# CliMA/ClimaOcean.jl

Measured on AMD Instinct MI355X. Metric: flux-kernel surface cells/s (update_state!: JRA55 interp + similarity-theory fluxes + net fluxes), higher is better.
Workload: dtype f64

## Files before the change

### climaocean.jl_amd/coflux/abi.py

```python
import ctypes as C
import os

import numpy as np

ABI_VERSION = 5
COMM_ID_BYTES = 128
PEER_HANDLE_BYTES = 64
HALO_NONE, HALO_RCCL, HALO_PEER = 0, 1, 2
FOLD_CENTER, FOLD_X_FACE, FOLD_Y_FACE = 0, 1, 2
SKIN_EXPLICIT, SKIN_SEMI_IMPLICIT, SKIN_LINEARISED = 0, 1, 2

SIMILARITY_LOGARITHMIC, SIMILARITY_COARE_LOGARITHMIC = 0, 1
STABILITY_EDSON2013, STABILITY_SHEBA, STABILITY_LARGE_YEAGER = 0, 1, 2
ROUGHNESS_CONSTANT, ROUGHNESS_CHARNOCK, ROUGHNESS_WIND_CHARNOCK = 0, 1, 2
SCALAR_ROUGHNESS_CONSTANT, SCALAR_ROUGHNESS_REYNOLDS = 0, 1
VISCOSITY_CONSTANT, VISCOSITY_TEMPERATURE_DEPENDENT = 0, 1
STOP_CONVERGENCE, STOP_FIXED = 0, 1
FORMULATION_SIMILARITY, FORMULATION_LARGE_YEAGER = 0, 1
VELOCITY_RELATIVE, VELOCITY_WIND = 0, 1
MASK_NONE, MASK_U8, MASK_BOTTOM_HEIGHT = 0, 1, 2
ALBEDO_CONSTANT, ALBEDO_LATITUDE_DEPENDENT = 0, 1
OPT_SOLVER, OPT_TRIP_HINTS, OPT_FUSED_NET, OPT_ICE_ORBIT_SHORTCUT, OPT_MERGED_PREFETCH = 0, 3, 6, 7, 9
OPT_INTERP_TILE_CAP, OPT_AO_CHUNK = 1, 4
OPT_INTERP_TILE_ROWS = 15
# ... 285 lines not shown
    "cf_device_alloc", "cf_device_free", "cf_h2d", "cf_d2h",
    "cf_interpolate_atmosphere_state", "cf_compute_atmosphere_ocean_fluxes",
    "cf_compute_net_ocean_fluxes", "cf_update_state", "cf_normalize_salinity_flux",
    "cf_default_sea_ice_params", "cf_set_sea_ice_formulation", "cf_compute_atmosphere_sea_ice_fluxes",
    "cf_compute_net_sea_ice_fluxes", "cf_update_state_sea_ice",
    "cf_time_stage", "cf_time_copy", "cf_profile_enable", "cf_profile_read",
    "cf_comm_unique_id", "cf_comm_init", "cf_comm_destroy", "cf_halo_exchange_rows",
    "cf_peer_halo_export", "cf_peer_halo_connect", "cf_halo_exchange_rows_peer", "cf_peer_halo_stats", "cf_fold_north_halo",
    "cf_time_steps", "cf_prefetch_atmosphere_state",
    "cf_default_sea_ice_albedo_params", "cf_set_sea_ice_albedo", "cf_compute_sea_ice_albedo",
    "cf_default_ice_ocean_params", "cf_compute_sea_ice_ocean_fluxes",
    "cf_interpolate_land_freshwater", "cf_set_land_freshwater", "cf_materialize_salinity_restoring",
    "cf_window_create", "cf_window_destroy", "cf_window_host_buffer", "cf_window_wait_slot", "cf_window_commit",
    "cf_window_upload", "cf_window_find", "cf_window_source",
    "cf_ensure_chunk_table", "cf_debug_chunk_table", "cf_debug_interp_grid", "cf_debug_land_zero_launches", "cf_solver_path", "cf_solver_iteration_path", "cf_solver_latency_layout", "cf_comm_count", "cf_build_stamp", "cf_discard_prefetched_atmosphere_state",
    "cf_debug_prefetch_stats",
    "cf_average_create", "cf_average_destroy", "cf_average_reset", "cf_average_collect", "cf_average_weight", "cf_attach_average",
    "cf_average_create_derived", "cf_average_create_budget", "cf_attach_average_slot",
    "cf_integrals_create", "cf_integrals_destroy", "cf_integrals_collect", "cf_integrals_count", "cf_integrals_read",
    "cf_integrals_reset", "cf_attach_integrals",
    "cf_monitor_create", "cf_monitor_destroy", "cf_monitor_collect", "cf_monitor_count", "cf_monitor_read", "cf_monitor_status",
    "cf_monitor_reset", "cf_attach_monitor",
    "cf_climatology_create", "cf_climatology_destroy", "cf_climatology_reset", "cf_climatology_collect", "cf_climatology_weights",
    "cf_climatology_extremes", "cf_calendar_bin", "cf_attach_climatology",
    "cf_regrid_create", "cf_regrid_destroy", "cf_regrid_apply",
    "cf_prepare_coupled_step", "cf_time_steps_coupled",
    "cf_checkpoint_create", "cf_checkpoint_destroy", "cf_checkpoint_add_array", "cf_checkpoint_add_average", "cf_checkpoint_add_climatology",
    "cf_checkpoint_add_integrals", "cf_checkpoint_add_monitor", "cf_checkpoint_set_host_blob", "cf_checkpoint_capture", "cf_checkpoint_wait",
    "cf_checkpoint_restore", "cf_checkpoint_verify", "cf_checkpoint_hash", "cf_checkpoint_host_blob",
)

# ... 101 lines not shown
    lib.cf_peer_halo_connect.argtypes = [vp, vp, vp, C.c_int, C.c_int]
    lib.cf_halo_exchange_rows_peer.argtypes = [vp, C.POINTER(vp), C.c_int, C.c_int]
    lib.cf_fold_north_halo.argtypes = [vp, C.POINTER(vp), C.POINTER(C.c_int), C.POINTER(C.c_double), C.c_int, C.c_int]
    lib.cf_time_steps.argtypes = [
        vp, C.c_int64, C.c_int, C.POINTER(RunSchedule), C.POINTER(AtmosSource), C.POINTER(InterpWeights),
        C.POINTER(InterfaceFluxes), C.POINTER(SeaIceFields), C.POINTER(NetOceanFluxes)]
    lib.cf_prepare_coupled_step.argtypes = [vp, C.POINTER(CoupledPrepare)]
    lib.cf_time_steps_coupled.argtypes = [
        vp, C.c_int64, C.c_int, C.POINTER(RunSchedule), C.POINTER(AtmosSource), C.POINTER(InterpWeights),
        C.POINTER(InterfaceFluxes), C.POINTER(SeaIceFields), C.POINTER(NetOceanFluxes), C.POINTER(CoupledStep)]
    lib.cf_prefetch_atmosphere_state.argtypes = [vp, C.POINTER(AtmosSource), C.POINTER(InterpWeights), C.POINTER(ExchangeFields)]
    lib.cf_ensure_chunk_table.argtypes = [vp, vp]
    lib.cf_debug_chunk_table.argtypes = [vp, C.POINTER(C.c_int), C.POINTER(C.c_int), C.c_int, C.POINTER(C.c_int), C.POINTER(C.c_int)]
    lib.cf_debug_interp_grid.argtypes = [vp, C.POINTER(C.c_int), C.POINTER(C.c_int)]
    lib.cf_debug_land_zero_launches.argtypes = [vp, C.POINTER(C.c_int)]
    lib.cf_solver_path.argtypes = [vp, C.POINTER(C.c_int), C.POINTER(C.c_int)]
    lib.cf_default_sea_ice_albedo_params.argtypes = [C.POINTER(SeaIceAlbedoParams)]
    lib.cf_set_sea_ice_albedo.argtypes = [vp, C.POINTER(SeaIceAlbedoParams)]
    lib.cf_compute_sea_ice_albedo.argtypes = [vp, C.POINTER(SeaIceAlbedoParams), vp, vp, vp, vp]
    lib.cf_default_ice_ocean_params.argtypes = [C.POINTER(IceOceanParams)]
    lib.cf_compute_sea_ice_ocean_fluxes.argtypes = [vp, C.POINTER(IceOceanParams), C.POINTER(OceanSurface), vp, vp, vp,
                                                    C.POINTER(IceOceanFluxes)]
    lib.cf_interpolate_land_freshwater.argtypes = [vp, C.POINTER(LandSource), C.POINTER(InterpWeights), vp]
    lib.cf_set_land_freshwater.argtypes = [vp, vp]
    lib.cf_materialize_salinity_restoring.argtypes = [vp, C.c_double, vp, C.POINTER(OceanSurface), vp]
    lib.cf_window_create.argtypes = [vp, C.c_int32, C.c_int32, C.c_int32, C.POINTER(vp)]
    lib.cf_window_destroy.argtypes = [vp]
    lib.cf_window_host_buffer.argtypes = [vp, C.c_int32, C.c_int32]
    lib.cf_window_host_buffer.restype = C.POINTER(C.c_float)
    lib.cf_window_wait_slot.argtypes = [vp, C.c_int32]
# ... 34 lines not shown
        getattr(lib, "cf_checkpoint_add_" + kind).argtypes = [vp, C.c_char_p, vp]
    lib.cf_checkpoint_set_host_blob.argtypes = [vp, vp, C.c_size_t]
    lib.cf_checkpoint_capture.argtypes = [vp]
    lib.cf_checkpoint_wait.argtypes = [vp, C.POINTER(vp), C.POINTER(C.c_size_t)]
    lib.cf_checkpoint_restore.argtypes = [vp, vp, C.c_size_t]
    lib.cf_checkpoint_verify.argtypes = [vp, C.c_size_t]
    lib.cf_checkpoint_hash.argtypes = [vp, C.c_size_t, C.POINTER(C.c_uint64)]
    lib.cf_checkpoint_host_blob.argtypes = [vp, C.c_size_t, C.POINTER(vp), C.POINTER(C.c_size_t)]
    for name in EXPORTED_SYMBOLS:
        fn = getattr(lib, name)
        if name not in ("cf_last_error", "cf_device_alloc", "cf_window_host_buffer", "cf_build_stamp"):
            fn.restype = C.c_int
    if path is None:
        _lib = lib
    return lib
```

### climaocean.jl_amd/coflux/runtime.py

```python
import ctypes as C

import numpy as np
import torch

from . import abi

EXCHANGE_NAMES = ("u", "v", "T", "p", "q", "Qs", "Ql", "Mp")
FLUX_NAMES = ("sensible_heat", "latent_heat", "water_vapor", "x_momentum", "y_momentum", "temperature")
FLUX_OPTIONAL = ("friction_velocity", "temperature_scale", "humidity_scale")
NET_NAMES = ("u", "v", "T", "S", "shortwave_surface_flux", "upwelling_longwave",
             "downwelling_longwave", "downwelling_shortwave")
ICE_NAMES = ("concentration", "interface_heat", "salt_flux", "x_stress", "y_stress")


class CofluxError(RuntimeError):
    pass


def _ptr(t):
    return None if t is None else C.c_void_p(t.data_ptr())


def _is_field(t, ctx, dtype=torch.float64):
    return t.is_cuda and t.is_contiguous() and tuple(t.shape) == ctx.shape and dtype in (None, t.dtype)
# ... 258 lines not shown
                                               counts.ctypes.data_as(C.POINTER(C.c_int)), capacity, C.byref(n), C.byref(valid))
            if rc != 0 and n.value + 1 > capacity:
                capacity = n.value + 1
                continue
            self._check(rc, "cf_debug_chunk_table")
            return begins[:n.value + 1].copy(), counts[:n.value].copy(), bool(valid.value)

    def debug_interp_grid(self):
        rows, blocks = C.c_int(), C.c_int()
        self._check(self.lib.cf_debug_interp_grid(self._h, C.byref(rows), C.byref(blocks)), "cf_debug_interp_grid")
        return rows.value, blocks.value

    def debug_land_zero_launches(self):
        n = C.c_int()
        self._check(self.lib.cf_debug_land_zero_launches(self._h, C.byref(n)), "cf_debug_land_zero_launches")
        return n.value

    def solver_path(self):
        lean, fused = C.c_int(), C.c_int()
        self._check(self.lib.cf_solver_path(self._h, C.byref(lean), C.byref(fused)), "cf_solver_path")
        return bool(lean.value), fused.value

    def solver_iteration_path(self):
        path = C.c_int()
        self._check(self.lib.cf_solver_iteration_path(self._h, C.byref(path)), "cf_solver_iteration_path")
        return path.value

    def solver_latency_layout(self):
        layout = C.c_int()
        self._check(self.lib.cf_solver_latency_layout(self._h, C.byref(layout)), "cf_solver_latency_layout")
# ... 687 lines not shown
```

### climaocean.jl_amd/csrc/coflux_abi.cpp

```cpp
#include "coflux_ctx.hpp"

static thread_local std::string g_error;
static RcclApi g_rccl;

int cf_fail(cf_ctx* ctx, int code, const char* fmt, ...) {
    char buf[1024];
    va_list ap;
    va_start(ap, fmt);
    vsnprintf(buf, sizeof buf, fmt, ap);
    va_end(ap);
    g_error = buf;
    if (ctx) {
        std::lock_guard<std::mutex> lock(ctx->error_mutex);
        ctx->error = buf;
    }
    return code;
}

static int wait_for_halos(cf_ctx* ctx);
int cf_flush_deferred_prefetch(cf_ctx* ctx);

static bool roughness_ok(const cf_roughness& r, bool scalar) {
    if (scalar) {
        if (r.kind == CF_SCALAR_ROUGHNESS_CONSTANT) return r.constant_length > 0;
// ... 699 lines not shown
    if (out->struct_size != (int32_t)sizeof(cf_prefetch_stats))
        return fail(ctx, CF_ERR_INVALID, "cf_prefetch_stats.struct_size = %d, library expects %zu", out->struct_size, sizeof(cf_prefetch_stats));
    *out = ctx->prefetch_stats;
    out->struct_size = (int32_t)sizeof(cf_prefetch_stats);
    out->pending = ctx->deferred.valid ? 1 : 0;
    for (const auto& p : ctx->prefetch) out->pending += p.valid ? 1 : 0;
    return CF_OK;
}

int cf_debug_land_zero_launches(cf_ctx* ctx, int* launches) {
    if (!ctx || !launches) return fail(ctx, CF_ERR_INVALID, "cf_debug_land_zero_launches: bad arguments");
    *launches = ctx->step_loop.zero_launches;
    return CF_OK;
}

int cf_debug_interp_grid(cf_ctx* ctx, int* rows, int* blocks) {
    if (!ctx || !rows || !blocks) return fail(ctx, CF_ERR_INVALID, "cf_debug_interp_grid: bad arguments");
    interpolate_grid(ctx->launch, ctx->grid, rows, blocks);
    return CF_OK;
}

static bool interp_tile_fits(const cf_ctx* ctx, size_t lds_bytes) {
    return ctx->launch.interp_cap > 0 && (size_t)4 * CF_JRA55_NVARS * (size_t)ctx->launch.interp_cap * sizeof(double) <= lds_bytes;
}

static bool net_fluxes_fused(const cf_ctx* ctx) {
    const bool lean = ctx->fast.specialization == SOLVER_OCEAN_LEAN && ctx->launch.solver == CF_SOLVER_TABLES;
    const bool fixed_trips = ctx->fast.specialization == SOLVER_LY && ctx->launch.solver == CF_SOLVER_TABLES;
    return (ctx->fused_net == 1 || (ctx->fused_net == 2 && (lean || fixed_trips))) && ctx->launch.solver == CF_SOLVER_TABLES &&
           ctx->dev.albedo_kind == CF_ALBEDO_CONSTANT;
// ... 135 lines not shown
            H.blocks = 2 * H.F.n;
            H.chunk_south = ctx->launch.chunk_south;
            H.chunk_north = ctx->launch.chunk_north;
            H.wait_south = ctx->peer.south != nullptr;
            H.wait_north = ctx->peer.north != nullptr;
            halo = &halo_rider;
        } else {
            CHECK(cf_peer_halo_launch_now(ctx, &ctx->halo_request.F, ctx->halo_request.rows));
        }
    }
    const unsigned way = 1u | (fuse ? 2u : 0u) | (ride ? 4u : 0u) | ((unsigned)ctx->fast.specialization << 3);
    const bool knows = ctx->launch.solver == CF_SOLVER_TABLES;
    const bool keep_land = knows && (ctx->land_zeros == 2 || (ctx->land_zeros == 1 && ctx->step_loop.open && ctx->step_loop.last_way == way));
    LaunchCfg L = ctx->launch;
    L.keep_land = keep_land ? 1 : 0;
    if (ride) {
        HIP_TRY(ctx, make_ocean_rider(L, ctx->dev, ctx->fast, ctx->grid, ocean, atmos, fluxes, ice, net, ctx->d_land_freshwater,
                                      ocean_rider));
    } else if (tail) {
        int rows = 4, blocks = 1;
        interpolate_grid(L, ctx->grid, &rows, &blocks);
        if (tail_lean)
            HIP_TRY(ctx, launch_ao_fluxes_lean(ctx->stream, L, ctx->dev, ctx->fast, ctx->grid, ocean, atmos, fluxes, ice, net,
                                               ctx->d_land_freshwater, &ctx->deferred.src, &ctx->deferred.w, &ctx->deferred.out, rows, blocks, halo));
        else
            HIP_TRY(ctx, launch_ly_fluxes_with_tail(ctx->stream, L, ctx->dev, ctx->fast, ctx->grid, ocean, atmos, fluxes, ice, net,
                                                    ctx->d_land_freshwater, &ctx->deferred.src, &ctx->deferred.w, &ctx->deferred.out, rows, blocks));
        CHECK(deferred_went_out_on_main(ctx, &ctx->prefetch_stats.launched_tail));
    } else
    HIP_TRY(ctx, launch_ao_fluxes(ctx->stream, L, ctx->dev, ctx->fast, ctx->grid, ocean, atmos, fluxes,
// ... 610 lines not shown
```

### climaocean.jl_amd/csrc/coflux_ctx.hpp

```cpp
#pragma once
#include <dlfcn.h>
#include <hip/hip_runtime.h>
#include <rccl/rccl.h>

#include <algorithm>
#include <cmath>
#include <cstdarg>
#include <cstdint>
#include <cstdio>
#include <cstdlib>
#include <cstring>
#include <mutex>
#include <string>
#include <vector>

#include "../../include/coflux.h"
#include "coflux_fast.hpp"
#include "coflux_kernel_types.hpp"
#include "coflux_kernels.h"
#include "coflux_owned.hpp"
#include "coflux_tables.h"

using namespace coflux;

#ifndef CF_LAND_ZEROS_DEFAULT
#define CF_LAND_ZEROS_DEFAULT 1
#endif
static_assert(CF_LAND_ZEROS_DEFAULT == 0 || CF_LAND_ZEROS_DEFAULT == 1, "the experiment value is not a default");

struct RcclApi {
    void* handle = nullptr;
    ncclResult_t (*GetUniqueId)(ncclUniqueId*) = nullptr;
    ncclResult_t (*CommInitRank)(ncclComm_t*, int, ncclUniqueId, int) = nullptr;
    ncclResult_t (*CommDestroy)(ncclComm_t) = nullptr;
    ncclResult_t (*GroupStart)() = nullptr;
    ncclResult_t (*GroupEnd)() = nullptr;
    ncclResult_t (*Send)(const void*, size_t, ncclDataType_t, int, ncclComm_t, hipStream_t) = nullptr;
    ncclResult_t (*Recv)(void*, size_t, ncclDataType_t, int, ncclComm_t, hipStream_t) = nullptr;
    const char* (*GetErrorString)(ncclResult_t) = nullptr;
    ncclResult_t (*AllReduce)(const void*, void*, size_t, ncclDataType_t, ncclRedOp_t, ncclComm_t, hipStream_t) = nullptr;
    ncclResult_t (*CommCount)(const ncclComm_t, int*) = nullptr;
    ncclResult_t (*CommUserRank)(const ncclComm_t, int*) = nullptr;
    ncclResult_t (*CommCuDevice)(const ncclComm_t, int*) = nullptr;
// ... 127 lines not shown
    cf::DeviceBuffer<int> d_peer_status;
    int halo_in_launch = 0;
    unsigned long long halo_in_launch_count = 0;
    cf::DeviceBuffer<unsigned long long> d_halo_counters;
    unsigned long long halo_expect_sent[2] = {0, 0}, halo_expect_done[2] = {0, 0};
    struct HaloRequest {
        bool valid = false;
        PeerFields F{};
        int rows = 0;
    } halo_request;
    int land_zeros = CF_LAND_ZEROS_DEFAULT;
    struct StepLoop {
        bool open = false;
        unsigned last_way = 0;
        int zero_launches = 0;
    } step_loop;
    ncclComm_t comm = nullptr;
    int rank = 0, nranks = 1;
    std::vector<cf::Event> prof_events;
    int prof_capacity = 0, prof_count = 0;
    std::vector<cf_child*> children;
    std::vector<struct cf_checkpoint*> checkpoints;
    struct AverageSlot {
        cf_average* handle = nullptr;
        int32_t stride = 1;
        double step_weight = 0.0;
        bool collects(int64_t step) const { return handle && (step + 1) % stride == 0; }
    } averages[CF_ATTACHED_AVERAGES_MAX];
    SeriesAttachment<cf_integrals> integrals;
    SeriesAttachment<cf_monitor> monitor;
    ClimatologyAttachment climatology;
// ... 113 lines not shown
```

### climaocean.jl_amd/csrc/coflux_interp_tiles.hpp

```cpp
#pragma once
#include <hip/hip_runtime.h>

#include <climits>

#include "coflux_interp_cell.hpp"
#include "coflux_kernel_types.hpp"

namespace coflux {

constexpr int IT_WAVES = 4;

template <bool MIN>
__device__ __forceinline__ int wave_reduce(int v) {
    auto op = [](int a, int b) { return MIN ? min(a, b) : max(a, b); };
    v = op(v, __builtin_amdgcn_update_dpp(v, v, 0xb1, 0xf, 0xf, false));
    v = op(v, __builtin_amdgcn_update_dpp(v, v, 0x4e, 0xf, 0xf, false));
    v = op(v, __builtin_amdgcn_update_dpp(v, v, 0x141, 0xf, 0xf, false));
    v = op(v, __builtin_amdgcn_update_dpp(v, v, 0x140, 0xf, 0xf, false));
    const int a = __builtin_amdgcn_readlane(v, 0), b = __builtin_amdgcn_readlane(v, 16);
    const int c = __builtin_amdgcn_readlane(v, 32), d = __builtin_amdgcn_readlane(v, 48);
    return op(op(a, b), op(c, d));
}
__device__ __forceinline__ int wave_min(int v) { return wave_reduce<true>(v); }
__device__ __forceinline__ int wave_max(int v) { return wave_reduce<false>(v); }

__device__ __forceinline__ void wave_lds_sync() {
    __builtin_amdgcn_fence(__ATOMIC_ACQ_REL, "wavefront");
    __builtin_amdgcn_wave_barrier();
}

template <int ROWS>
__device__ __forceinline__ void interpolate_tiles(const SourceDesc& S, const WeightDesc& Wt, const GridDesc& G, const Exchange& E, int cap,
                                                  int block, int nblocks) {
    extern __shared__ __attribute__((aligned(16))) char smem[];
    const int lane = threadIdx.x & 63, wave = threadIdx.x >> 6;
    double* tile = reinterpret_cast<double*>(smem) + (size_t)wave * CF_JRA55_NVARS * cap;

    const int wx = G.nx + 2 * G.ring, wy = G.ny + 2 * G.ring;
    const int tiles_x = (wx + 63) / 64, tiles_y = (wy + ROWS - 1) / ROWS;
    const int ntiles = tiles_x * tiles_y;
    const size_t plane = (size_t)S.ns_x * S.ns_y;
    const size_t off1 = (size_t)S.level1 * plane, off2 = (size_t)S.level2 * plane;
    const int half = S.ns_x / 2;
    const bool rotate = Wt.cos_rot != nullptr && Wt.sin_rot != nullptr;

    for (int t = block * IT_WAVES + wave; t < ntiles; t += nblocks * IT_WAVES) {
        const int ty = t / tiles_x, tx = t - ty * tiles_x;
        const int i = tx * 64 + lane - G.ring;
        const int ic = min(i, G.nx + G.ring - 1);

        int d0[ROWS], di[ROWS], j0[ROWS], j1[ROWS];
        double xi[ROWS], eta[ROWS];
        int lo = INT_MAX, hi = INT_MIN, jlo = INT_MAX, jhi = INT_MIN, ref = 0;
#pragma unroll
        for (int r = 0; r < ROWS; ++r) {
            const int jc = min(ty * ROWS + r - G.ring, G.ny + G.ring - 1);
            const size_t k = cell_index(G, ic, jc);
            const double fi = Wt.separable ? Wt.fi[ic + G.hx] : Wt.fi[k];
            const double fj = Wt.separable ? Wt.fj[jc + G.hy] : Wt.fj[k];
            const double ti = trunc(fi), tj = trunc(fj);
            xi[r] = fi - floor(fi);
            eta[r] = fj - floor(fj);
            const int i0 = (int)ti;
            di[r] = fi > 0.0 ? 1 : (fi < 0.0 ? -1 : 0);
            const int ja = (int)tj;
            const int jb = ja + (fj > 0.0 ? 1 : (fj < 0.0 ? -1 : 0));
            j0[r] = min(max(ja, 0), S.ns_y - 1);
            j1[r] = min(max(jb, 0), S.ns_y - 1);
            if (r == 0) ref = __shfl(i0, 0);
            d0[r] = wrap_index(i0 - ref + half, S.ns_x) - half;
            lo = min(lo, min(d0[r], d0[r] + di[r]));
            hi = max(hi, max(d0[r], d0[r] + di[r]));
            jlo = min(jlo, min(j0[r], j1[r]));
            jhi = max(jhi, max(j0[r], j1[r]));
        }
        lo = wave_min(lo);
        hi = wave_max(hi);
        jlo = wave_min(jlo);
        jhi = wave_max(jhi);
        const int W = hi - lo + 1, H = jhi - jlo + 1, WH = W * H;
        const bool fits = WH <= cap && W <= S.ns_x;

        if (fits) {
            const float inv_W = 1.0f / (float)W;
            for (int rem = lane; rem < WH; rem += 64) {
                const int y = (int)(((float)rem + 0.5f) * inv_W);
                const int x = rem - y * W;
                const size_t off = (size_t)(jlo + y) * S.ns_x + wrap_index(ref + lo + x, S.ns_x);
#pragma unroll
// ... 16 lines not shown
                    const double* p = tile + v * cap;
                    val[v] = bilinear(w00, w01, w10, w11, p[o00], p[o01], p[o00 + di[r]], p[o01 + di[r]]);
                }
            } else {
                const int is0 = wrap_index(ref + d0[r], S.ns_x), is1 = wrap_index(ref + d0[r] + di[r], S.ns_x);
                const size_t g00 = (size_t)j0[r] * S.ns_x + is0, g10 = (size_t)j0[r] * S.ns_x + is1;
                const size_t g01 = (size_t)j1[r] * S.ns_x + is0, g11 = (size_t)j1[r] * S.ns_x + is1;
#pragma unroll
                for (int v = 0; v < CF_JRA55_NVARS; ++v) {
                    const float* a = S.data[v] + off1;
                    const float* b = S.data[v] + off2;
                    val[v] = bilinear(w00, w01, w10, w11, blend_levels(a[g00], b[g00], S.tf), blend_levels(a[g01], b[g01], S.tf),
                                      blend_levels(a[g10], b[g10], S.tf), blend_levels(a[g11], b[g11], S.tf));
                }
            }
            if (i < G.nx + G.ring && j < G.ny + G.ring) {
                const size_t k = cell_index(G, i, j);
                double ua = val[CF_JRA55_UAS], va = val[CF_JRA55_VAS];
                if (rotate) {
                    const double cs = Wt.cos_rot[k], sn = Wt.sin_rot[k];
                    const double ui = ua * cs + va * sn;
                    va = -ua * sn + va * cs;
                    ua = ui;
                }
                E.u[k] = ua;
                E.v[k] = va;
                E.T[k] = val[CF_JRA55_TAS];
                E.p[k] = val[CF_JRA55_PSL];
                E.q[k] = val[CF_JRA55_HUSS];
                E.Qs[k] = val[CF_JRA55_RSDS];
                E.Ql[k] = val[CF_JRA55_RLDS];
                E.Mp[k] = val[CF_JRA55_PRRA] + val[CF_JRA55_PRSN];
            }
        }
        wave_lds_sync();
    }
}

}
```

### climaocean.jl_amd/csrc/coflux_kernels.h

```cpp
#pragma once
#include <hip/hip_runtime.h>

#include <cstdlib>

#include "coflux_device.hpp"

namespace coflux {

inline bool experiments_enabled() {
    static const bool enabled = [] {
        const char* e = std::getenv("COFLUX_EXPERIMENTS");
        return e != nullptr && e[0] == '1';
    }();
    return enabled;
}

struct LoopParams;
struct IceParams;
struct HaloRider;

struct LaunchCfg {
    int solver;
    int interp_cap;
    int interp_rows;
    int ao_chunk;
    int cu_count;
    const double* d_tables;
    const DevParams* d_params;
    uint8_t* d_trip;
    const int* d_chunk_begins;
    int n_chunks;
    int chunk_south, chunk_north;
    const uint32_t* d_wet_pos;
    uint32_t* d_lean_sorted;
    const int* d_lean_info;
    int lean_hints;
    int certified;
    int latency_layout;
    int keep_land;
};

bool lean_line_applies(const LaunchCfg& L, const LoopParams& C, bool coare);

bool lean_certified_applies(const LaunchCfg& L, const LoopParams& C);

hipError_t launch_interpolate(hipStream_t st, const LaunchCfg& L, const GridDesc& G, const cf_atmos_source* s,
                              const cf_interp_weights* w, const cf_exchange_fields* e);
hipError_t launch_ao_fluxes(hipStream_t st, const LaunchCfg& L, const DevParams& P, const LoopParams& C,
                            const GridDesc& G, const cf_ocean_surface* o, const cf_exchange_fields* e,
                            const cf_interface_fluxes* f, const cf_sea_ice_fields* ice = nullptr,
                            const cf_net_ocean_fluxes* net = nullptr, const double* land = nullptr);
hipError_t launch_net_stress(hipStream_t st, const DevParams& P, const GridDesc& G, const cf_ocean_surface* o,
                             const cf_interface_fluxes* f, const cf_sea_ice_fields* ice, const cf_net_ocean_fluxes* n,
                             bool keep_land = false);
// ... 214 lines not shown
```

### climaocean.jl_amd/csrc/coflux_lean_kernel.hpp

```cpp
#pragma once
#include <hip/hip_runtime.h>

#include "coflux_halo_device.hpp"
#include "coflux_interp_tiles.hpp"
#include "coflux_lean.hpp"
#include "coflux_certified.hpp"
#include "coflux_solver_shared.hpp"

namespace coflux {

constexpr int LEAN_WAVES = 3;

struct LeanArgs {
    LoopParams L;
    GridDesc G;
    OceanIn O;
    Exchange E;
    FluxOut F;
    const double* g_tab;
    const DevParams* g_params;
    uint32_t* sorted;
    const int* info;
    const int* chunk_begins;
    double z_surface;
    long long mask_kind;
    double T_offset;
    unsigned long long wx_reciprocal;
    long long sort_enabled;
    IceIn I;
    NetOut N;
    SourceDesc S;
    WeightDesc Wt;
    Exchange E_next;
    long long n_chunks;
    long long tail_blocks, tail_rows, tail_cap;
    long long tail_pos;
    HaloRider H;
    long long keep_land;
};
typedef const LeanArgs __attribute__((address_space(4)))* LeanArgsPtr;

hipError_t launch_ao_lean_line(hipStream_t st, bool coare, bool fuse, bool tail, bool halo, int blocks, const LeanArgs& A);

__device__ __forceinline__ LeanArgsPtr opaque(LeanArgsPtr p) {
    asm volatile("" : "+s"(p));
    return p;
}

__device__ __forceinline__ unsigned lean_mix(unsigned idx) { return (idx * 0x9e3779b1u) ^ ((idx * 0x85ebca6bu) >> 15); }
__device__ __forceinline__ unsigned lean_sum(unsigned idx) { return idx * 0xc2b2ae35u + 0x27d4eb2fu; }

constexpr int LEAN_LIST_OFFSET = TABLE_BYTES;
constexpr int LEAN_OFFSET_BITS = 24;
// ... 48 lines not shown
            peer_halo_rider(M, K->H.F.ptr[f], f, dir, K->H.rows, K->H.seq, K->H.counters, K->H.expect_sent[dir], K->H.status, Gh, BLOCK,
                            reinterpret_cast<int*>(smem_h));
            return;
        }
        chunk -= nh;
    }
    if constexpr (TAIL) {
        static_assert(BLOCK == 64 * IT_WAVES, "a tail workgroup is an interpolation workgroup");
        const int nb = (int)K->tail_blocks, ipos = (int)K->tail_pos;
        if (chunk >= ipos && chunk < ipos + nb) {
            const SourceDesc S = kread(&K->S);
            const WeightDesc Wt = kread(&K->Wt);
            const GridDesc Gt = kread(&K->G);
            const Exchange En = kread(&K->E_next);
            const int b = chunk - ipos, cap = (int)K->tail_cap, rows = (int)K->tail_rows;
            if (rows == 4) interpolate_tiles<4>(S, Wt, Gt, En, cap, b, nb);
            else if (rows == 2) interpolate_tiles<2>(S, Wt, Gt, En, cap, b, nb);
            else interpolate_tiles<1>(S, Wt, Gt, En, cap, b, nb);
            return;
        }
        if (chunk >= ipos) chunk -= nb;
    }
    if constexpr (HALO) {
        const int cs = K->H.chunk_south, cn = K->H.chunk_north, nc = (int)K->n_chunks;
        if (K->H.blocks > 0) {
            if (cs <= cn) {
                const int inner = cn - cs;
                chunk = chunk < inner ? cs + chunk : (chunk - inner < cs ? chunk - inner : cn + (chunk - inner - cs));
            }
            wait_south = K->H.wait_south != 0 && chunk < cs;
            wait_north = K->H.wait_north != 0 && chunk >= cn && chunk < nc;
        }
    }
// ... 402 lines not shown
```

### climaocean.jl_amd/csrc/coflux_solver.hip

```cpp
#include <hip/hip_runtime.h>

#include <cstring>

#include "coflux_solver_shared.hpp"
#include "coflux_lean.hpp"
#include "coflux_lean_kernel.hpp"

namespace coflux {

int wet_list_stride();
struct Geom {
    static constexpr int CHUNK = AO_CHUNK;
    static constexpr int COUNTERS_OFFSET = TABLE_DOUBLES * 8 + CHUNK * 4;
    static constexpr int PARAMS_OFFSET = COUNTERS_OFFSET + 16 + 2 * 64 * 4;
    static constexpr int LDS_BYTES = PARAMS_OFFSET + (int)sizeof(DevParams);
};
constexpr int AO_LAYER_1 = AO_CHUNK < 1024 ? AO_CHUNK : 1024, AO_LAYER_2 = AO_CHUNK < 768 ? AO_CHUNK : 768, AO_LAYER_3 = 512;
static_assert(AO_LAYER_1 <= AO_CHUNK && AO_LAYER_1 >= AO_LAYER_2 && AO_LAYER_2 >= AO_LAYER_3, "layer sizes");
static_assert(AO_BINS == 64, "Geom::PARAMS_OFFSET spells the bin count out");
static_assert(Geom::LDS_BYTES <= 53760, "three narrow solver workgroups must fit the CU's 160 KB of LDS");


constexpr int AO_MAX_ROUNDS = 8;
struct ChunkRounds {
// ... 232 lines not shown
__device__ __forceinline__ void ao_flux_fast_body(SolverArgsPtr K_in, const int block) {
    constexpr int BLOCK = AO_BLOCK, CHUNK = Geom::CHUNK;
    SolverArgsPtr K = opaque(K_in);
    if constexpr (TAIL) {
        static_assert(BLOCK == 64 * IT_WAVES, "a tail workgroup is an interpolation workgroup");
        const int nch = (int)K->n_chunks;
        if (block >= nch) {
            int b = block - nch;
            const int nb = (int)K->tail_blocks;
            const GridDesc Gt = kread(&K->G);
            if (b < nb) {
                const SourceDesc S = kread(&K->Si);
                const WeightDesc Wt = kread(&K->Wi);
                const Exchange En = kread(&K->E_next);
                const int cap = (int)K->tail_cap, rows = (int)K->tail_rows;
                if (rows == 4) interpolate_tiles<4>(S, Wt, Gt, En, cap, b, nb);
                else if (rows == 2) interpolate_tiles<2>(S, Wt, Gt, En, cap, b, nb);
                else interpolate_tiles<1>(S, Wt, Gt, En, cap, b, nb);
                return;
            }
            b -= nb;
            const int idx = b * 256 + (int)threadIdx.x;
            if (idx >= Gt.nx * Gt.ny) return;
            const DevParams& Po = *K->stress_params;
            const IceIn I = kread(&K->stress_ice);
            const void* smask = K->stress_mask;
            const double* __restrict__ rtx = K->rtx;
            const double* __restrict__ rty = K->rty;
            const int j = idx / Gt.nx;
            const size_t k = cell_index(Gt, idx - j * Gt.nx, j);
            const size_t kw = k - 1, ks = k - (size_t)Gt.sj;
            const bool wet = cell_is_wet(Po, smask, k);
            const double aice = I.conc ? I.conc[k] : 0.0;
// ... 494 lines not shown
        C.specialization != SOLVER_LY)
        return hipErrorInvalidValue;
    if ((size_t)IT_WAVES * CF_JRA55_NVARS * L.interp_cap * sizeof(double) > (size_t)Geom::LDS_BYTES) return hipErrorInvalidValue;
    const IceIn I = make_ice_in(ice, land);
    const NetOut N = make_net_out(net);
    SolverArgs A{C, G, make_ocean(o), make_exchange(e), make_fluxes(f), L.d_tables, L.d_params, WetLists{L.d_wet_pos, nullptr},
                 L.d_chunk_begins, I, N, IceStateIn{}, IceParams{}, P.z_surface, P.mask_kind, P.T_offset, row_reciprocal(G.nx + 2 * G.ring)};
    A.Si = make_source(next_src);
    A.Wi = make_weights(w);
    A.E_next = make_exchange(next_out);
    A.n_chunks = L.n_chunks;
    A.tail_blocks = tail_blocks;
    A.tail_rows = tail_rows;
    A.tail_cap = L.interp_cap;
    A.keep_land = L.keep_land;
    hipLaunchKernelGGL((ao_flux_fast_kernel<true, SOLVER_LY, true, true>), dim3(L.n_chunks + tail_blocks), dim3(AO_BLOCK),
                       Geom::LDS_BYTES, st, A);
    return hipGetLastError();
}

hipError_t launch_ao_fluxes(hipStream_t st, const LaunchCfg& L, const DevParams& P, const LoopParams& C,
                            const GridDesc& G, const cf_ocean_surface* o, const cf_exchange_fields* e,
                            const cf_interface_fluxes* f, const cf_sea_ice_fields* ice, const cf_net_ocean_fluxes* net,
                            const double* land) {
    if (L.solver == CF_SOLVER_LIBM) return net ? hipErrorInvalidValue : launch_ao_fluxes_libm(st, P, G, o, e, f);
    if (C.specialization == SOLVER_OCEAN_LEAN) {
        if (!L.d_lean_info) return hipErrorInvalidValue;
        return launch_ao_fluxes_lean(st, L, P, C, G, o, e, f, ice, net, land);
    }
    OceanIn O = make_ocean(o);
// ... 142 lines not shown
```

### climaocean.jl_amd/csrc/coflux_solver_lean.hip

```cpp
#include <hip/hip_runtime.h>

#include <cstring>

#include "coflux_lean_kernel.hpp"

namespace coflux {

template <bool COARE, bool FUSE, bool TAIL = false, bool CERT = false>
__global__ __launch_bounds__(AO_BLOCK, LEAN_WAVES) void ao_lean_kernel(LeanArgs unused_by_name) {
    ao_lean_body<COARE, FUSE, TAIL, CERT>((LeanArgsPtr)__builtin_amdgcn_kernarg_segment_ptr(), (int)blockIdx.x);
}

template <bool COARE>
__global__ __launch_bounds__(AO_BLOCK, LEAN_WAVES) void ao_lean_halo_kernel(LeanArgs unused_by_name) {
    ao_lean_body<COARE, true, true, false, false, true>((LeanArgsPtr)__builtin_amdgcn_kernarg_segment_ptr(), (int)blockIdx.x);
}

__global__ __launch_bounds__(256) void lean_list_build_kernel(const uint32_t* __restrict__ wet_pos, const int* __restrict__ begins, int stride,
                                                              uint32_t* __restrict__ sorted, int* __restrict__ info) {
    __shared__ unsigned sx[4], sy[4];
    __shared__ int sn[4];
    const int chunk = blockIdx.x, lane = threadIdx.x & 63, wave = threadIdx.x >> 6;
    const int begin = begins[chunk];
    unsigned hx = 0, hy = 0;
// ... 99 lines not shown
    const bool cert = lean_certified_applies(L, C);
    const bool tail = next_out != nullptr;
    int blocks = L.n_chunks;
    if (tail) {
        if (!net || !next_src || !w || L.interp_cap <= 0 || tail_blocks <= 0) return hipErrorInvalidValue;
        const size_t tile_lds = (size_t)IT_WAVES * CF_JRA55_NVARS * L.interp_cap * sizeof(double);
        if (tile_lds > (size_t)LeanGeom<AO_BLOCK>::LDS_BYTES) return hipErrorInvalidValue;
        A.S = make_source(next_src);
        A.Wt = make_weights(w);
        A.E_next = make_exchange(next_out);
        A.n_chunks = L.n_chunks;
        A.tail_blocks = tail_blocks;
        A.tail_rows = tail_rows;
        A.tail_cap = L.interp_cap;
        A.tail_pos = L.n_chunks;
        blocks += tail_blocks;
    }
    const bool riders = halo != nullptr && halo->blocks > 0;
    if (riders) {
        if (!tail || !lean_halo_rides(L, C) || halo->F.n < 1 || halo->blocks != 2 * halo->F.n) return hipErrorInvalidValue;
        A.H = *halo;
        blocks += halo->blocks;
    }
    if (lean_line_applies(L, C, coare)) return launch_ao_lean_line(st, coare, net != nullptr, tail, riders, blocks, A);
    if (riders) {
        if (coare) hipLaunchKernelGGL((ao_lean_halo_kernel<true>), dim3(blocks), dim3(AO_BLOCK), LeanGeom<AO_BLOCK>::LDS_BYTES, st, A);
        else hipLaunchKernelGGL((ao_lean_halo_kernel<false>), dim3(blocks), dim3(AO_BLOCK), LeanGeom<AO_BLOCK>::LDS_BYTES, st, A);
        return hipGetLastError();
    }
#define CF_LEAN_LAUNCH(COARE_, FUSE_, TAIL_, CERT_) \
// ... 19 lines not shown
```

### climaocean.jl_amd/csrc/coflux_solver_shared.hpp

```cpp
#pragma once
#include <hip/hip_runtime.h>

#include "coflux_fast.hpp"
#include "coflux_kernel_types.hpp"
#include "coflux_kernels.h"
#include "coflux_interp_tiles.hpp"

namespace coflux {

constexpr int TABLE_BYTES = TABLE_DOUBLES * 8;
constexpr int AO_BLOCK = 256;
constexpr int AO_CHUNK = 1280;
constexpr int AO_BINS = 64;
constexpr int AO_WET_COST = 64;

template <bool FUSE_NET>
__device__ __forceinline__ void zero_cell(const LoopParams& L, double T_offset, const GridDesc& G, const FluxOut& F,
                                          const NetOut& N, size_t k, int i, int j) {
    CellFluxes Z{};
    Z.Ts_ocean = -T_offset;
    Z.iterations = L.fixed ? L.maxiter : 0;
    store_fluxes(F, k, Z);
    if constexpr (FUSE_NET) {
        if (i >= 0 && i < G.nx && j >= 0 && j < G.ny) store_net_cell(N, k, NetCell{});
// ... 29 lines not shown
    unsigned long long wx_reciprocal;
    SourceDesc Si;
    WeightDesc Wi;
    Exchange E_next;
    long long n_chunks, tail_blocks, tail_rows, tail_cap;
    long long stress_blocks;
    const DevParams* stress_params;
    const void* stress_mask;
    const double* rtx;
    const double* rty;
    IceIn stress_ice;
    double* tau_x;
    double* tau_y;
    NetIceOut NI;
    long long keep_land;
};
typedef const SolverArgs __attribute__((address_space(4)))* SolverArgsPtr;

template <class T>
__device__ __forceinline__ T kread(const __attribute__((address_space(4))) T* p) {
    static_assert(sizeof(T) % 8 == 0, "argument bundles are made of 8-byte words");
    T v;
    const __attribute__((address_space(4))) unsigned long long* src = (const __attribute__((address_space(4))) unsigned long long*)p;
    unsigned long long* dst = reinterpret_cast<unsigned long long*>(&v);
#pragma unroll
    for (size_t n = 0; n < sizeof(T) / 8; ++n) dst[n] = src[n];
    return v;
}

__device__ __forceinline__ double gload(const double* base, unsigned byte_off) {
// ... 44 lines not shown
```

### climaocean.jl_amd/csrc/coflux_steps.cpp

```cpp
#include <map>
#include <optional>

#include "coflux_series.hpp"

static std::mutex g_peer_mutex;
static std::map<std::string, std::pair<char*, int>> g_peer_local;

static int ensure_aux_stream(cf_ctx* ctx) {
    if (ctx->aux.stream) return CF_OK;
    HIP_TRY(ctx, hipSetDevice(ctx->device));
    cf_ctx::AuxLane lane;
    HIP_TRY(ctx, lane.stream.create());
    HIP_TRY(ctx, lane.ev_gate.create(hipEventDisableTiming));
    for (cf::Event& e : lane.done) HIP_TRY(ctx, e.create(hipEventDisableTiming));
    ctx->aux = std::move(lane);
    for (int k = 0; k < 2; ++k) ctx->prefetch[k].done = ctx->aux.done[k].get();
    return CF_OK;
}

int cf_launch_prefetch(cf_ctx* ctx, const cf_atmos_source* src, const cf_interp_weights* w, const cf_exchange_fields* out) {
    cf_ctx::Prefetch* rec = ctx->prefetch_slot(out->u);
    if (!rec) return fail(ctx, CF_ERR_INVALID, "two prefetched atmosphere states are already pending");
    if (!ctx->deferred.gated) HIP_TRY(ctx, hipEventRecord(ctx->aux.ev_gate.get(), ctx->stream));
    ctx->deferred.gated = false;
// ... 411 lines not shown
                CHECK(cf_flush_deferred_prefetch(ctx));
                if (!ctx->prefetch_slot(a0->u)) return fail(ctx, CF_ERR_INVALID, "two prefetched atmosphere states are already pending");
                CHECK(supersede_states(ctx, a0->u));
                HIP_TRY(ctx, launch_interpolate(ctx->stream, ctx->launch, ctx->grid, &s0, w, a0));
                ++ctx->prefetch_stats.requests;
                ctx->deferred.src = s0;
                ctx->deferred.w = *w;
                ctx->deferred.out = *a0;
                CHECK(deferred_went_out_on_main(ctx, &ctx->prefetch_stats.launched_own));
            } else {
                CHECK(request_prefetch(ctx, &s0, w, a0, false));
            }
        }
    }
    std::optional<LandZeroScope> land_zero_scope;
    if (!K) land_zero_scope.emplace(ctx);
    for (int64_t step = first_step; step < first_step + nsteps; ++step) {
        const cf_ocean_surface* o = &S->ocean_states[step % S->n_ocean_states];
        double* rows[4] = {const_cast<double*>(o->T), const_cast<double*>(o->S), const_cast<double*>(o->u),
                           const_cast<double*>(o->v)};
        if (S->halo_backend == CF_HALO_RCCL)
            CHECK(cf_halo_exchange_rows(ctx, rows, 4, S->halo_rows));
        else if (S->halo_backend == CF_HALO_PEER) {
            if (ctx->halo_in_launch && ctx->peer_connected && 4 <= ctx->peer_max_fields && S->halo_rows <= ctx->peer_max_rows &&
                S->halo_rows <= ctx->grid.ny) {
                ctx->halo_request.F = PeerFields{};
                ctx->halo_request.F.n = 4;
                for (int f = 0; f < 4; ++f) ctx->halo_request.F.ptr[f] = rows[f];
                ctx->halo_request.rows = S->halo_rows;
                ctx->halo_request.valid = true;
            } else {
                CHECK(cf_halo_exchange_rows_peer(ctx, rows, 4, S->halo_rows));
// ... 61 lines not shown
```

### include/coflux.h

```cpp
#ifndef COFLUX_H
#define COFLUX_H

#include <stddef.h>
#include <stdint.h>

#ifdef __cplusplus
extern "C" {
#endif

#define CF_ABI_VERSION 5

#define CF_OK 0
#define CF_ERR_INVALID (-1)
#define CF_ERR_HIP (-2)
#define CF_ERR_NODEVICE (-3)
#define CF_ERR_COMM (-4)

typedef struct cf_ctx cf_ctx;

typedef struct cf_grid {
    int32_t nx, ny;
    int32_t hx, hy;
    int32_t ring;
    int32_t reserved;
// ... 224 lines not shown
#define CF_OPT_ICE_FREE_CELLS 12
#define CF_ICE_FREE_ITERATE 0
#define CF_OPT_LATENCY_LAYOUT 13
#define CF_ICE_FREE_ZERO 1
#define CF_OPT_HALO_IN_SOLVER_LAUNCH 14
#define CF_OPT_INTERP_TILE_ROWS 15
#define CF_SOLVER_TABLES 0
#define CF_SOLVER_LIBM 1
int cf_set_option(cf_ctx* ctx, int option, int value);
int cf_solver_iteration_path(cf_ctx* ctx, int* path);
int cf_solver_latency_layout(cf_ctx* ctx, int* layout);
int cf_debug_eval(cf_ctx* ctx, int function, int n, const double* d_x, double* d_y);
int cf_debug_chunk_plan(long long total_cost, int cu_count, int forced_wet_per_chunk, int* out, int capacity);
int cf_debug_chunk_table(cf_ctx* ctx, int* begins, int* wet_counts, int capacity, int* n_chunks, int* lists_valid);
int cf_debug_land_zero_launches(cf_ctx* ctx, int* launches);
int cf_debug_interp_grid(cf_ctx* ctx, int* rows, int* blocks);
int cf_sync(cf_ctx* ctx);

void* cf_device_alloc(cf_ctx* ctx, size_t bytes);
int cf_device_free(cf_ctx* ctx, void* d_ptr);
int cf_h2d(cf_ctx* ctx, void* d_dst, const void* h_src, size_t bytes);
int cf_d2h(cf_ctx* ctx, void* h_dst, const void* d_src, size_t bytes);


int cf_interpolate_atmosphere_state(cf_ctx* ctx, const cf_atmos_source* src,
                                    const cf_interp_weights* w, const cf_exchange_fields* out);

int cf_compute_atmosphere_ocean_fluxes(cf_ctx* ctx, const cf_ocean_surface* ocean,
                                       const cf_exchange_fields* atmos,
                                       const cf_interface_fluxes* out);
// ... 477 lines not shown
```

Before: 10.23 billion.

## Skip land cells in pipelined interpolation tail when next step's solver ignores them

Inside the fused solver kernels, the interpolation tail that prefetches the next step's atmosphere now reads the ocean land mask and writes only wet cells. Whole tiles whose cells are all land are skipped by one wave-wide ballot. A step-position rule decides when this is safe: the next two pipelined steps must exist and no collectors may be attached, otherwise land values could be observed. This saves interpolation arithmetic and stores over land, at the cost of extra mask loads per tile and more bookkeeping of the step-loop state.

```diff
diff --git a/climaocean.jl_amd/coflux/abi.py b/climaocean.jl_amd/coflux/abi.py
--- a/climaocean.jl_amd/coflux/abi.py
+++ b/climaocean.jl_amd/coflux/abi.py
@@ -323,7 +323,7 @@
     "cf_window_create", "cf_window_destroy", "cf_window_host_buffer", "cf_window_wait_slot", "cf_window_commit",
     "cf_window_upload", "cf_window_find", "cf_window_source",
     "cf_ensure_chunk_table", "cf_debug_chunk_table", "cf_debug_interp_grid", "cf_debug_land_zero_launches", "cf_solver_path", "cf_solver_iteration_path", "cf_solver_latency_layout", "cf_comm_count", "cf_build_stamp", "cf_discard_prefetched_atmosphere_state",
-    "cf_debug_prefetch_stats",
+    "cf_debug_prefetch_stats", "cf_debug_rider_land_rule", "cf_debug_rider_land_skips",
     "cf_average_create", "cf_average_destroy", "cf_average_reset", "cf_average_collect", "cf_average_weight", "cf_attach_average",
     "cf_average_create_derived", "cf_average_create_budget", "cf_attach_average_slot",
     "cf_integrals_create", "cf_integrals_destroy", "cf_integrals_collect", "cf_integrals_count", "cf_integrals_read",
@@ -455,6 +455,8 @@
     lib.cf_debug_chunk_table.argtypes = [vp, C.POINTER(C.c_int), C.POINTER(C.c_int), C.c_int, C.POINTER(C.c_int), C.POINTER(C.c_int)]
     lib.cf_debug_interp_grid.argtypes = [vp, C.POINTER(C.c_int), C.POINTER(C.c_int)]
     lib.cf_debug_land_zero_launches.argtypes = [vp, C.POINTER(C.c_int)]
+    lib.cf_debug_rider_land_rule.argtypes = [C.c_longlong, C.c_int, C.c_int, C.POINTER(C.c_int), C.c_int]
+    lib.cf_debug_rider_land_skips.argtypes = [vp, C.POINTER(C.c_int)]
     lib.cf_solver_path.argtypes = [vp, C.POINTER(C.c_int), C.POINTER(C.c_int)]
     lib.cf_default_sea_ice_albedo_params.argtypes = [C.POINTER(SeaIceAlbedoParams)]
     lib.cf_set_sea_ice_albedo.argtypes = [vp, C.POINTER(SeaIceAlbedoParams)]
@@ -519,3 +521,10 @@
     if path is None:
         _lib = lib
     return lib
+
+
+def rider_land_rule(first_step, nsteps, pipeline):
+    out = (C.c_int * max(nsteps, 1))()
+    if load_library().cf_debug_rider_land_rule(first_step, nsteps, pipeline, out, len(out)) != 0:
+        raise ValueError(f"cf_debug_rider_land_rule({first_step}, {nsteps}, {pipeline}): bad arguments")
+    return list(out[:nsteps])
diff --git a/climaocean.jl_amd/coflux/runtime.py b/climaocean.jl_amd/coflux/runtime.py
--- a/climaocean.jl_amd/coflux/runtime.py
+++ b/climaocean.jl_amd/coflux/runtime.py
@@ -296,6 +296,11 @@
     def debug_land_zero_launches(self):
         n = C.c_int()
         self._check(self.lib.cf_debug_land_zero_launches(self._h, C.byref(n)), "cf_debug_land_zero_launches")
+        return n.value
+
+    def debug_rider_land_skips(self):
+        n = C.c_int()
+        self._check(self.lib.cf_debug_rider_land_skips(self._h, C.byref(n)), "cf_debug_rider_land_skips")
         return n.value
 
     def solver_path(self):
diff --git a/climaocean.jl_amd/csrc/coflux_abi.cpp b/climaocean.jl_amd/csrc/coflux_abi.cpp
--- a/climaocean.jl_amd/csrc/coflux_abi.cpp
+++ b/climaocean.jl_amd/csrc/coflux_abi.cpp
@@ -737,6 +737,22 @@
     return CF_OK;
 }
 
+int cf_debug_rider_land_rule(long long first_step, int nsteps, int pipeline, int* skips, int capacity) {
+    if (first_step < 0 || nsteps < 0 || pipeline < 0 || pipeline > CF_PIPELINE_CONTINUING || !skips || capacity < nsteps)
+        return fail(nullptr, CF_ERR_INVALID, "cf_debug_rider_land_rule: bad arguments");
+    for (int n = 0; n < nsteps; ++n) {
+        const int64_t step = first_step + n;
+        skips[n] = !rider_exists(step, first_step, nsteps, pipeline) ? -1 : (rider_may_skip_land(step, first_step, nsteps, pipeline) ? 1 : 0);
+    }
+    return CF_OK;
+}
+
+int cf_debug_rider_land_skips(cf_ctx* ctx, int* riders) {
+    if (!ctx || !riders) return fail(ctx, CF_ERR_INVALID, "cf_debug_rider_land_skips: bad arguments");
+    *riders = ctx->step_loop.rider_skips;
+    return CF_OK;
+}
+
 int cf_debug_interp_grid(cf_ctx* ctx, int* rows, int* blocks) {
     if (!ctx || !rows || !blocks) return fail(ctx, CF_ERR_INVALID, "cf_debug_interp_grid: bad arguments");
     interpolate_grid(ctx->launch, ctx->grid, rows, blocks);
@@ -902,6 +918,11 @@
     const bool keep_land = knows && (ctx->land_zeros == 2 || (ctx->land_zeros == 1 && ctx->step_loop.open && ctx->step_loop.last_way == way));
     LaunchCfg L = ctx->launch;
     L.keep_land = keep_land ? 1 : 0;
+    const cf_ctx::StepLoop& loop = ctx->step_loop;
+    const bool rider_skips = tail && loop.open && ctx->rider_land_skip != 0 && ctx->land_zeros != 0 && !ctx->collectors_attached() &&
+                             rider_may_skip_land(loop.step, loop.first_step, loop.nsteps, loop.pipeline);
+    L.rider_skip_land = rider_skips ? 1 : 0;
+    if (rider_skips) ++ctx->step_loop.rider_skips;
     if (ride) {
         HIP_TRY(ctx, make_ocean_rider(L, ctx->dev, ctx->fast, ctx->grid, ocean, atmos, fluxes, ice, net, ctx->d_land_freshwater,
                                       ocean_rider));
diff --git a/climaocean.jl_amd/csrc/coflux_ctx.hpp b/climaocean.jl_amd/csrc/coflux_ctx.hpp
--- a/climaocean.jl_amd/csrc/coflux_ctx.hpp
+++ b/climaocean.jl_amd/csrc/coflux_ctx.hpp
@@ -27,6 +27,18 @@
 #define CF_LAND_ZEROS_DEFAULT 1
 #endif
 static_assert(CF_LAND_ZEROS_DEFAULT == 0 || CF_LAND_ZEROS_DEFAULT == 1, "the experiment value is not a default");
+#ifndef CF_RIDER_LAND_SKIP_DEFAULT
+#define CF_RIDER_LAND_SKIP_DEFAULT 1
+#endif
+static_assert(CF_RIDER_LAND_SKIP_DEFAULT == 0 || CF_RIDER_LAND_SKIP_DEFAULT == 1, "on or off");
+
+inline bool rider_exists(int64_t t, int64_t first_step, int nsteps, int pipeline) {
+    if (pipeline == 0 || t < first_step || t >= first_step + nsteps) return false;
+    return t + 1 < first_step + nsteps || pipeline == CF_PIPELINE_CONTINUING;
+}
+inline bool rider_may_skip_land(int64_t step, int64_t first_step, int nsteps, int pipeline) {
+    return rider_exists(step, first_step, nsteps, pipeline) && rider_exists(step + 2, first_step, nsteps, pipeline);
+}
 
 struct RcclApi {
     void* handle = nullptr;
@@ -184,7 +196,16 @@
         bool open = false;
         unsigned last_way = 0;
         int zero_launches = 0;
+        int64_t first_step = 0, step = 0;
+        int nsteps = 0, pipeline = 0;
+        int rider_skips = 0;
     } step_loop;
+    int rider_land_skip = CF_RIDER_LAND_SKIP_DEFAULT;
+    bool collectors_attached() const {
+        for (const auto& slot : averages)
+            if (slot.handle) return true;
+        return climatology.handle || integrals.handle || monitor.handle;
+    }
     ncclComm_t comm = nullptr;
     int rank = 0, nranks = 1;
     std::vector<cf::Event> prof_events;
diff --git a/climaocean.jl_amd/csrc/coflux_interp_tiles.hpp b/climaocean.jl_amd/csrc/coflux_interp_tiles.hpp
--- a/climaocean.jl_amd/csrc/coflux_interp_tiles.hpp
+++ b/climaocean.jl_amd/csrc/coflux_interp_tiles.hpp
@@ -29,9 +29,16 @@
     __builtin_amdgcn_wave_barrier();
 }
 
-template <int ROWS>
-__device__ __forceinline__ void interpolate_tiles(const SourceDesc& S, const WeightDesc& Wt, const GridDesc& G, const Exchange& E, int cap,
-                                                  int block, int nblocks) {
+struct TileLand {
+    const void* mask = nullptr;
+    int kind = CF_MASK_NONE;
+    double z_surface = 0.0;
+    bool skip = false;
+};
+
+template <int ROWS, bool SKIP>
+__device__ __forceinline__ void interpolate_tiles_impl(const SourceDesc& S, const WeightDesc& Wt, const GridDesc& G, const Exchange& E, int cap,
+                                                       int block, int nblocks, const TileLand& land) {
     extern __shared__ __attribute__((aligned(16))) char smem[];
     const int lane = threadIdx.x & 63, wave = threadIdx.x >> 6;
     double* tile = reinterpret_cast<double*>(smem) + (size_t)wave * CF_JRA55_NVARS * cap;
@@ -43,6 +50,11 @@
     const size_t off1 = (size_t)S.level1 * plane, off2 = (size_t)S.level2 * plane;
     const int half = S.ns_x / 2;
     const bool rotate = Wt.cos_rot != nullptr && Wt.sin_rot != nullptr;
+    typedef const __attribute__((address_space(1))) unsigned* GlobalWords;
+    const int mask_kind = land.mask == nullptr ? CF_MASK_NONE : land.kind;
+    const unsigned long long mbase = mask_kind == CF_MASK_NONE ? (unsigned long long)Wt.fi : (unsigned long long)land.mask;
+    const unsigned mstride = mask_kind == CF_MASK_NONE ? 0u : (mask_kind == CF_MASK_U8 ? 1u : 8u);
+    const unsigned mhi_step = mask_kind == CF_MASK_BOTTOM_HEIGHT ? 4u : 0u;
 
     for (int t = block * IT_WAVES + wave; t < ntiles; t += nblocks * IT_WAVES) {
         const int ty = t / tiles_x, tx = t - ty * tiles_x;
@@ -52,12 +64,19 @@
         int d0[ROWS], di[ROWS], j0[ROWS], j1[ROWS];
         double xi[ROWS], eta[ROWS];
         int lo = INT_MAX, hi = INT_MIN, jlo = INT_MAX, jhi = INT_MIN, ref = 0;
+        unsigned raw_lo[ROWS], raw_hi[ROWS], raw_shift = 0;
 #pragma unroll
         for (int r = 0; r < ROWS; ++r) {
             const int jc = min(ty * ROWS + r - G.ring, G.ny + G.ring - 1);
             const size_t k = cell_index(G, ic, jc);
             const double fi = Wt.separable ? Wt.fi[ic + G.hx] : Wt.fi[k];
             const double fj = Wt.separable ? Wt.fj[jc + G.hy] : Wt.fj[k];
+            if constexpr (SKIP) {
+                const unsigned long long a = mbase + (unsigned long long)k * mstride;
+                raw_shift |= ((unsigned)a & 3u) << (2 * r);
+                raw_lo[r] = *(GlobalWords)(a & ~3ull);
+                raw_hi[r] = *(GlobalWords)((a & ~3ull) + mhi_step);
+            }
             const double ti = trunc(fi), tj = trunc(fj);
             xi[r] = fi - floor(fi);
             eta[r] = fj - floor(fj);
@@ -73,6 +92,20 @@
             hi = max(hi, max(d0[r], d0[r] + di[r]));
             jlo = min(jlo, min(j0[r], j1[r]));
             jhi = max(jhi, max(j0[r], j1[r]));
+        }
+        unsigned wet = 0;
+        if constexpr (SKIP) {
+#pragma unroll
+            for (int r = 0; r < ROWS; ++r) asm volatile("" : "+v"(raw_lo[r]), "+v"(raw_hi[r]));
+#pragma unroll
+            for (int r = 0; r < ROWS; ++r) {
+                const bool m = mask_kind == CF_MASK_NONE ? true
+                               : mask_kind == CF_MASK_U8 ? ((raw_lo[r] >> (8 * ((raw_shift >> (2 * r)) & 3u))) & 0xffu) != 0
+                                                         : !(land.z_surface <= __hiloint2double((int)raw_hi[r], (int)raw_lo[r]));
+                const bool inside = i < G.nx + G.ring && ty * ROWS + r - G.ring < G.ny + G.ring;
+                wet |= (m && inside ? 1u : 0u) << r;
+            }
+            if (__builtin_amdgcn_ballot_w64(wet != 0u) == 0ull) continue;
         }
         lo = wave_min(lo);
         hi = wave_max(hi);
@@ -119,7 +152,7 @@
                                       blend_levels(a[g10], b[g10], S.tf), blend_levels(a[g11], b[g11], S.tf));
                 }
             }
-            if (i < G.nx + G.ring && j < G.ny + G.ring) {
+            if (SKIP ? (wet >> r & 1u) != 0u : (i < G.nx + G.ring && j < G.ny + G.ring)) {
                 const size_t k = cell_index(G, i, j);
                 double ua = val[CF_JRA55_UAS], va = val[CF_JRA55_VAS];
                 if (rotate) {
@@ -142,4 +175,16 @@
     }
 }
 
+template <int ROWS>
+__device__ __forceinline__ void interpolate_tiles(const SourceDesc& S, const WeightDesc& Wt, const GridDesc& G, const Exchange& E, int cap,
+                                                  int block, int nblocks) {
+    interpolate_tiles_impl<ROWS, false>(S, Wt, G, E, cap, block, nblocks, TileLand{});
 }
+template <int ROWS>
+__device__ __forceinline__ void interpolate_tiles(const SourceDesc& S, const WeightDesc& Wt, const GridDesc& G, const Exchange& E, int cap,
+                                                  int block, int nblocks, const TileLand& land) {
+    if (land.skip) interpolate_tiles_impl<ROWS, true>(S, Wt, G, E, cap, block, nblocks, land);
+    else interpolate_tiles_impl<ROWS, false>(S, Wt, G, E, cap, block, nblocks, land);
+}
+
+}
diff --git a/climaocean.jl_amd/csrc/coflux_kernels.h b/climaocean.jl_amd/csrc/coflux_kernels.h
--- a/climaocean.jl_amd/csrc/coflux_kernels.h
+++ b/climaocean.jl_amd/csrc/coflux_kernels.h
@@ -38,6 +38,7 @@
     int certified;
     int latency_layout;
     int keep_land;
+    int rider_skip_land;
 };
 
 bool lean_line_applies(const LaunchCfg& L, const LoopParams& C, bool coare);
diff --git a/climaocean.jl_amd/csrc/coflux_lean_kernel.hpp b/climaocean.jl_amd/csrc/coflux_lean_kernel.hpp
--- a/climaocean.jl_amd/csrc/coflux_lean_kernel.hpp
+++ b/climaocean.jl_amd/csrc/coflux_lean_kernel.hpp
@@ -37,6 +37,7 @@
     long long tail_pos;
     HaloRider H;
     long long keep_land;
+    long long tail_skip_land;
 };
 typedef const LeanArgs __attribute__((address_space(4)))* LeanArgsPtr;
 
@@ -115,9 +116,14 @@
             const GridDesc Gt = kread(&K->G);
             const Exchange En = kread(&K->E_next);
             const int b = chunk - ipos, cap = (int)K->tail_cap, rows = (int)K->tail_rows;
-            if (rows == 4) interpolate_tiles<4>(S, Wt, Gt, En, cap, b, nb);
-            else if (rows == 2) interpolate_tiles<2>(S, Wt, Gt, En, cap, b, nb);
-            else interpolate_tiles<1>(S, Wt, Gt, En, cap, b, nb);
+            TileLand land;
+            land.skip = K->tail_skip_land != 0;
+            land.mask = K->O.mask;
+            land.kind = (int)K->mask_kind;
+            land.z_surface = K->z_surface;
+            if (rows == 4) interpolate_tiles<4>(S, Wt, Gt, En, cap, b, nb, land);
+            else if (rows == 2) interpolate_tiles<2>(S, Wt, Gt, En, cap, b, nb, land);
+            else interpolate_tiles<1>(S, Wt, Gt, En, cap, b, nb, land);
             return;
         }
         if (chunk >= ipos) chunk -= nb;
diff --git a/climaocean.jl_amd/csrc/coflux_solver.hip b/climaocean.jl_amd/csrc/coflux_solver.hip
--- a/climaocean.jl_amd/csrc/coflux_solver.hip
+++ b/climaocean.jl_amd/csrc/coflux_solver.hip
@@ -270,9 +270,16 @@
                 const WeightDesc Wt = kread(&K->Wi);
                 const Exchange En = kread(&K->E_next);
                 const int cap = (int)K->tail_cap, rows = (int)K->tail_rows;
-                if (rows == 4) interpolate_tiles<4>(S, Wt, Gt, En, cap, b, nb);
-                else if (rows == 2) interpolate_tiles<2>(S, Wt, Gt, En, cap, b, nb);
-                else interpolate_tiles<1>(S, Wt, Gt, En, cap, b, nb);
+                TileLand land;
+                if constexpr (SPEC == SOLVER_LY) {
+                    land.skip = K->tail_skip_land != 0;
+                    land.mask = K->tail_mask;
+                    land.kind = (int)K->mask_kind;
+                    land.z_surface = K->z_surface;
+                }
+                if (rows == 4) interpolate_tiles<4>(S, Wt, Gt, En, cap, b, nb, land);
+                else if (rows == 2) interpolate_tiles<2>(S, Wt, Gt, En, cap, b, nb, land);
+                else interpolate_tiles<1>(S, Wt, Gt, En, cap, b, nb, land);
                 return;
             }
             b -= nb;
@@ -797,6 +804,8 @@
     A.tail_rows = tail_rows;
     A.tail_cap = L.interp_cap;
     A.keep_land = L.keep_land;
+    A.tail_skip_land = L.rider_skip_land;
+    A.tail_mask = o->mask;
     hipLaunchKernelGGL((ao_flux_fast_kernel<true, SOLVER_LY, true, true>), dim3(L.n_chunks + tail_blocks), dim3(AO_BLOCK),
                        Geom::LDS_BYTES, st, A);
     return hipGetLastError();
diff --git a/climaocean.jl_amd/csrc/coflux_solver_lean.hip b/climaocean.jl_amd/csrc/coflux_solver_lean.hip
--- a/climaocean.jl_amd/csrc/coflux_solver_lean.hip
+++ b/climaocean.jl_amd/csrc/coflux_solver_lean.hip
@@ -137,6 +137,7 @@
         A.tail_rows = tail_rows;
         A.tail_cap = L.interp_cap;
         A.tail_pos = L.n_chunks;
+        A.tail_skip_land = L.rider_skip_land;
         blocks += tail_blocks;
     }
     const bool riders = halo != nullptr && halo->blocks > 0;
diff --git a/climaocean.jl_amd/csrc/coflux_solver_shared.hpp b/climaocean.jl_amd/csrc/coflux_solver_shared.hpp
--- a/climaocean.jl_amd/csrc/coflux_solver_shared.hpp
+++ b/climaocean.jl_amd/csrc/coflux_solver_shared.hpp
@@ -67,6 +67,8 @@
     double* tau_y;
     NetIceOut NI;
     long long keep_land;
+    long long tail_skip_land;
+    const void* tail_mask;
 };
 typedef const SolverArgs __attribute__((address_space(4)))* SolverArgsPtr;
 
diff --git a/climaocean.jl_amd/csrc/coflux_steps.cpp b/climaocean.jl_amd/csrc/coflux_steps.cpp
--- a/climaocean.jl_amd/csrc/coflux_steps.cpp
+++ b/climaocean.jl_amd/csrc/coflux_steps.cpp
@@ -449,8 +449,14 @@
         }
     }
     std::optional<LandZeroScope> land_zero_scope;
-    if (!K) land_zero_scope.emplace(ctx);
+    if (!K) {
+        land_zero_scope.emplace(ctx);
+        ctx->step_loop.first_step = first_step;
+        ctx->step_loop.nsteps = nsteps;
+        ctx->step_loop.pipeline = S->pipeline;
+    }
     for (int64_t step = first_step; step < first_step + nsteps; ++step) {
+        ctx->step_loop.step = step;
         const cf_ocean_surface* o = &S->ocean_states[step % S->n_ocean_states];
         double* rows[4] = {const_cast<double*>(o->T), const_cast<double*>(o->S), const_cast<double*>(o->u),
                            const_cast<double*>(o->v)};
diff --git a/include/coflux.h b/include/coflux.h
--- a/include/coflux.h
+++ b/include/coflux.h
@@ -262,6 +262,8 @@
 int cf_debug_chunk_plan(long long total_cost, int cu_count, int forced_wet_per_chunk, int* out, int capacity);
 int cf_debug_chunk_table(cf_ctx* ctx, int* begins, int* wet_counts, int capacity, int* n_chunks, int* lists_valid);
 int cf_debug_land_zero_launches(cf_ctx* ctx, int* launches);
+int cf_debug_rider_land_rule(long long first_step, int nsteps, int pipeline, int* skips, int capacity);
+int cf_debug_rider_land_skips(cf_ctx* ctx, int* riders);
 int cf_debug_interp_grid(cf_ctx* ctx, int* rows, int* blocks);
 int cf_sync(cf_ctx* ctx);
 
```

After: 10.32 billion (median of 6 runs). No clear change (+0.9%).
